# DanHelmy/hdr-realtime-video-pipeline

Hardware: AMD Instinct MI355X
Metric: frames/sec (HDRTVNet++ AGCM+LE+HG fp16 3840x2160 + fused RGB48 post into the pinned host ring); p50 per-frame ms in p50_ms (higher is better)
Workload: dtype f16

## Files before the change

### hdr-realtime-video-pipeline_amd/csrc/api_graph.hip

```cpp
#include "api.h"

namespace hdrtv_host {

void Seq::conv(const std::string &key, const f16 *src0, int c0, const f16 *src1, int c1, int Hi, int Wi, int act, int mode, f16 *dst, int dstC, int Hd, int Wd, const f16 *res1, const f16 *res2, f16 *dst_full, f16 *dst_planar, const f16 *res_planar, const float *dotw, float *dst_dot, int s0_stride)
{
    if (!ok()) return;
    auto it = c->conv.find(key);
    if (it == c->conv.end()) { rc = fail(c, HDRTV_ESTATE, "no packed conv %s", key.c_str()); return; }
    const ConvLayer &L = it->second;
    ConvParams p;
    memset(&p, 0, sizeof p);
    p.src0 = src0; p.src1 = src1; p.c0 = c0; p.c1 = c1;
    p.s0_stride = s0_stride ? s0_stride : c0; p.s1_stride = c1;
    p.Hi = Hi; p.Wi = Wi;
    const int pad = L.ks / 2;
    p.Ho = (Hi + 2 * pad - L.ks) / L.stride + 1;
    p.Wo = (Wi + 2 * pad - L.ks) / L.stride + 1;
    p.wpk = wtp<f16>(c, L.wpk); p.scale = wtp<float>(c, L.scale); p.shift = wtp<float>(c, L.shift);
    p.CoutPad = L.coutPad; p.Cout = L.cout; p.act = act; p.mode = mode;
    p.dst = dst; p.dst_full = dst_full; p.dstC = dstC; p.Hd = Hd; p.Wd = Wd;
    p.res1 = res1; p.res2 = res2; p.dst_planar = dst_planar; p.res_planar = res_planar;
    p.dotw = dotw; p.dst_dot = dst_dot;
    if (c0 + c1 != L.cin) { rc = fail(c, HDRTV_ESTATE, "conv %s: channel mismatch", key.c_str()); return; }
    p.zeros = wtp<f16>(c, c->zeros_off);
// ... 548 lines not shown
    }
    q.conv32("LE.up_conv3.0", t5, nullptr, "", s.H1, s.W1, ACT_RELU, ST_PS, up3, 32, H, W, fea0);
    q.conv32("LE.HR_conv2", up3, cond1, "LE.SFT_layer2", H, W, ACT_RELU, ST_NHWC, f0b, 32, H, W);
    q.conv32("LE.conv_last", f0b, nullptr, "", H, W, ACT_NONE, ST_PLANAR3, nullptr, 0, H, W, nullptr, nullptr, out_planar, img);
    return q.rc;
}

size_t hg_need_plan(hdrtv_ctx *c, int Hp, int Wp, HgNeedParams &p)
{
    memset(&p, 0, sizeof p);
    p.Hp = Hp; p.Wp = Wp;
    constexpr int n_layers = (int)(sizeof hg_layers / sizeof hg_layers[0]);
    static_assert(n_layers + 1 <= HG_NEED_MAX_LAYERS && n_layers + 3 <= HG_NEED_MAX_TENSORS, "hg_need's tables are too small");
    constexpr int max_level = [] { int m = 0; for (const HgLayer &L : hg_layers) m = L.level > m ? L.level : m; return m; }();
    static_assert(max_level < HG_NEED_LEVELS, "hg_need's unit tables have too few levels");
    memcpy(p.lu, hg_need_unit_log2[c->var.at("hg_sparse") == 1 ? 1 : 2], sizeof p.lu);
    auto ncell = [&](int level) { return (((Hp >> level) + 15) / 16) * (((Wp >> level) + 15) / 16); };
    auto nwords = [&](int level) {
        size_t m = 0;
        for (const auto &tab : hg_need_unit_log2) {
            const int u = 1 << tab[level], rows = std::max(((Hp >> level) + u - 1) / u, ((Hp >> level) + 7) / 8);
            m = std::max(m, (size_t)rows * ((((Wp >> level) + u - 1) / u + 63) / 64));
        }
        return m;
    };
    const char *names[HG_NEED_MAX_TENSORS];
    int level[HG_NEED_MAX_TENSORS], nt = 0;
    auto tensor = [&](const char *name, int lev) {
        if (!name) name = "part";
        for (int i = 0; i < nt; ++i)
            if (!strcmp(names[i], name)) return i;
        names[nt] = name; level[nt] = lev;
        return nt++;
    };
    for (int i = 0; i < n_layers; ++i) {
        const HgLayer &L = hg_layers[i];
        HgNeedLayer &N = p.L[i + 1];
        N.level = L.level; N.ks = L.ks; N.tw = 16;
        N.mode = L.mode == ST_POOL ? 1 : (L.ps ? 2 : 0);
        N.in = tensor(L.in, L.level);
        N.skip = L.skip ? tensor(L.skip, L.level) : -1;
        N.out = tensor(L.out, L.out_level());
        N.th = L.ks == 3 && Seq::prw_tile_rows(c, L.mode, L.cout, Hp >> L.level, Wp >> L.level) == 8 ? 8 : 16;
    }
    const int nt_table = nt;
    {
        HgNeedLayer &N = p.L[0];
        N.level = 0; N.ks = 3; N.mode = 1;
        N.out = tensor(hg_layers[0].in, 1);
        N.in = tensor("img", 0);
        N.skip = -1;
        N.th = 8; N.tw = 32;
    }
    p.n_layers = n_layers + 1;
    bool seen[HG_NEED_MAX_TENSORS] = {};
    for (int i = p.n_layers - 1; i >= 0; --i) {
        HgNeedLayer &N = p.L[i];
        N.in_first = !seen[N.in];
        seen[N.in] = true;
        if (N.skip >= 0) { N.skip_first = !seen[N.skip]; seen[N.skip] = true; }
    }
    size_t off = 0;
    auto take = [&](size_t bytes) { const size_t o = off; off = (off + bytes + 15) & ~(size_t)15; return (int)o; };
    p.flags_off = take((size_t)ncell(0));
    take((size_t)ncell(0));
    for (int t = 0; t < nt_table; ++t)
        if (strcmp(names[t], "part")) take((size_t)ncell(level[t]));
    for (int i = 1; i <= n_layers; ++i) p.L[i].list_off = take(4 * (2 * (size_t)ncell(p.L[i].level) + 4));
    size_t scratch = 0;
    for (int t = 0; t < nt; ++t) scratch = std::max(scratch, nwords(level[t]));
    for (int t = 0; t < nt_table; ++t) {
        p.map_off[t] = take(8 * nwords(level[t]));
        if (!strcmp(names[t], "part")) p.flags_map = t;
    }
    for (int i = 0; i < p.n_layers; ++i) {
        p.L[i].out_chained = i + 1 < p.n_layers ? p.L[i + 1].in == p.L[i].out : p.L[i].out == p.flags_map;
        p.L[i].in_chained = i > 0 && p.L[i - 1].out == p.L[i].in;
    }
    p.scratch_words = (int)scratch;
    p.kbits_off = take(8 * scratch);
    p.tbits_off = take(8 * scratch);
    p.L[0].list_off = take(4 * (2 * (size_t)ncell(0) + 4));
    p.map_off[nt_table] = take(8 * nwords(0));
    return off;
}

int run_hg(hdrtv_ctx *c, Seq &q, const f16 *base, void *out, int out_f32, bool complete_taps)
{
    const Shapes s = shapes_for(c->H, c->W);
    const int Hp = s.Hp, Wp = s.Wp;
    f16 *img = q.wsp<f16>("hg.img");
    uint8_t *mask = q.wsp<uint8_t>("hg.mask");
    const bool sparse = !complete_taps && c->var.at("hg_sparse") != 0 && !c->hg_i8 && !c->var.at("final_recompute");
    HgNeedParams np;
    if (sparse) {
        hg_need_plan(c, Hp, Wp, np);
        np.base = q.wsp<unsigned char>("hg.need");
    }
    if (q.ws == c->lane_ws[0] && !complete_taps) {
        hipStreamCaptureStatus cap = hipStreamCaptureStatusNone;
        c->taps_partial = sparse;
        c->taps_replayable = sparse && hipStreamIsCapturing(q.s, &cap) == hipSuccess && cap != hipStreamCaptureStatusNone;
        c->taps_stream = q.s;
    }
    if (!complete_taps)
        q.chk(hg_prep_launch(base, s.H, s.W, Hp, Wp, img, mask, c->mask_r, 0.1f, q.s, sparse ? np.base + np.flags_off : nullptr), "hg_prep",
              "hg_prep", 0.0, 13.0 * Hp * Wp);
    if (sparse) q.chk(hg_need_launch(np, q.s), "hg_need", "hg_need", 0.0, 0.0);
    float *part = q.wsp<float>("hg.part");
    const bool light = !c->var.at("final_recompute");
    float *part2 = light ? q.wsp<float>("hg.part2") : nullptr;
    const f16 *w2frag = light ? wtp<f16>(c, c->hgf_wfrag) + 6 * 64 * 8 : nullptr;
    constexpr int n_layers = (int)(sizeof hg_layers / sizeof hg_layers[0]);
    const char *tn[3 * n_layers];
    void *tp[3 * n_layers];
    int nt = 0;
    auto tensor = [&](const char *name) -> void * {
        if (!name) return nullptr;
        for (int i = 0; i < nt; ++i)
            if (!strcmp(tn[i], name)) return tp[i];
        char key[32];
        snprintf(key, sizeof key, "%s%s", c->hg_i8 ? "hg8." : "hg.", name);
        tn[nt] = name;
        tp[nt] = q.wsp<void>(key);
        return tp[nt++];
    };
    const bool c1_list = sparse && light;
    q.c3("hg.conv1", img, Hp, Wp, ACT_RELU, nullptr, (f16 *)tensor(hg_layers[0].in), c->hg_q0_inv, c->hg_q0_zero, w2frag, part2,
         c1_list ? reinterpret_cast<const int *>(np.base + np.L[0].list_off) : nullptr, c1_list ? ((Hp + 7) / 8) * ((Wp + 31) / 32) : 0);
    char key[32];
    for (const HgLayer &L : hg_layers) {
        snprintf(key, sizeof key, "hg.%s", L.name);
        if (sparse) {
            const HgNeedLayer &N = np.L[&L - hg_layers + 1];
            q.need_list = reinterpret_cast<const int *>(np.base + N.list_off);
            q.need_th = N.th;
            q.need_total = (((Hp >> L.level) + N.th - 1) / N.th) * (((Wp >> L.level) + 15) / 16);
        }
        const int c1 = L.skip_cin, c0 = L.cin - c1, Hi = Hp >> L.level, Wi = Wp >> L.level;
        const int Ho = Hp >> L.out_level(), Wo = Wp >> L.out_level();
        const bool dot3 = L.mode == ST_PS_DOT3;
        const float *dotw = dot3 ? wtp<float>(c, c->hg_w10a) : nullptr;
        float *dst_dot = dot3 ? part : nullptr;
        if (c->hg_i8)
            q.conv8(key, (const int8_t *)tensor(L.in), c0, (const int8_t *)tensor(L.skip), c1, Hi, Wi, L.mode, tensor(L.out), L.out_c(), Ho, Wo, dotw, dst_dot);
        else
            q.conv(key, (const f16 *)tensor(L.in), c0, (const f16 *)tensor(L.skip), c1, Hi, Wi, L.act, L.mode, (f16 *)tensor(L.out), L.out_c(), Ho, Wo,
                   nullptr, nullptr, nullptr, nullptr, nullptr, dotw, dst_dot);
    }
    if (!q.ok() || complete_taps) return q.rc;
    const C3Layer &L1 = c->c3.at("hg.conv1");
    HgFinalFusedArgs fa;
    fa.img = img; fa.mask = mask; fa.part = part; fa.wfrag = wtp<f16>(c, c->hgf_wfrag);
    fa.scale = wtp<float>(c, L1.scale); fa.shift = wtp<float>(c, L1.shift);
    fa.b10 = wtp<float>(c, c->f32v.at("hg.b10"));
    fa.wl = wtp<float>(c, c->f32v.at("hg.wl")); fa.bl = wtp<float>(c, c->f32v.at("hg.bl"));
    fa.out = out; fa.out_f32 = out_f32; fa.H = s.H; fa.W = s.W; fa.Hp = Hp; fa.Wp = Wp;
    if (light)
        q.chk(hg_final_light_launch(fa, part2, q.s), "hg_final", "hg_final_light", (double)s.H * s.W * 6 * 3,
              (double)s.H * s.W * (6 + 1 + 32 + 3 * (out_f32 ? 4 : 2)));
#ifdef HDRTV_AB
    else
        q.chk(hg_final_fused_launch(fa, c->n_cu, q.s), "hg_final", "hg_final_fused", (double)Hp * Wp * (128 * 3 + 6 * 3),
              (double)s.H * s.W * (6 + 1 + 16 + 3 * (out_f32 ? 4 : 2)));
#endif
    return q.rc;
}

}
```

### hdr-realtime-video-pipeline_amd/csrc/api_util.hip

```cpp
#include "api.h"

namespace hdrtv_host {

int fail(hdrtv_ctx *c, int code, const char *fmt, ...)
{
    char buf[512];
    va_list ap;
    va_start(ap, fmt);
    vsnprintf(buf, sizeof buf, fmt, ap);
    va_end(ap);
    if (c) { std::lock_guard<std::mutex> lk(c->err_mu); c->err = buf; }
    return code;
}

namespace {
const std::pair<const char *, int> k_variants[] = {
    {"le_rows", 1},
    {"le_rows_min", 8},
    {"le_rows_i8", 1},
    {"le_rows_fq", 1},
    {"prw", 1},
    {"prw_i8", 1},
    {"pglds_nt_slow", 3},
    {"no_t16", 0},
    {"conv32_old", 0},
    {"conv32_nosplit", 0},
    {"conv32_nw", 0},
    {"no_c3fuse", 0},
    {"no_c3q8", 0},
    {"glds1_old", 0},
    {"hg_sparse", 2},
    {"final_recompute", 0},
    {"cond3_fused", 1},
    {"cond2_fused", 1},
    {"pre_split", 0},
    {"force_ncu", 0},
    {"light_wgs", 2},
    {"f32_narrow_below", 0},
    {"f32_mfma", 1},
};
const char *const k_ab_only[] = {"conv32_old", "conv32_nosplit", "conv32_nw", "glds1_old", "final_recompute"};
}
bool variant_allowed(const std::string &name, int value)
{
#ifdef HDRTV_AB
    (void)name; (void)value;
    return true;
#else
    if (value == 0) return true;
    for (const char *n : k_ab_only) if (name == n) return false;
    return true;
#endif
}
void variants_init(hdrtv_ctx *c)
{
    for (const auto &kv : k_variants) c->var[kv.first] = kv.second;
    const char *e = getenv("HDRTV_VARIANTS");
    if (!e) return;
    std::string str(e);
    size_t pos = 0;
    while (pos < str.size()) {
        size_t nx = str.find(',', pos);
        if (nx == std::string::npos) nx = str.size();
        const std::string one = str.substr(pos, nx - pos);
        const size_t eq = one.find('=');
        if (eq != std::string::npos) {
            auto it = c->var.find(one.substr(0, eq));
            if (it != c->var.end() && variant_allowed(it->first, atoi(one.c_str() + eq + 1))) it->second = atoi(one.c_str() + eq + 1);
        }
        pos = nx + 1;
    }
}

}
```

### hdr-realtime-video-pipeline_amd/csrc/hg_need.hip

```cpp
#include "launchers.h"

namespace {

constexpr int NT = 1024, LDS_WORDS = 2304;
using u64 = unsigned long long;

__constant__ u64 k_tile_bits[5] = {~0ull, 0x5555555555555555ull, 0x1111111111111111ull, 0x0101010101010101ull, 0x0001000100010001ull};

struct Map {
    int h, w, nw;
};
__device__ __forceinline__ Map map_of(const HgNeedParams &p, int level)
{
    const int lu = p.lu[level], r = (1 << lu) - 1;
    Map m;
    m.h = ((p.Hp >> level) + r) >> lu;
    m.w = ((p.Wp >> level) + r) >> lu;
    m.nw = (m.w + 63) >> 6;
    return m;
}
__device__ __forceinline__ u64 word(const u64 *b, const Map &m, int y, int wi)
{
    return (unsigned)y < (unsigned)m.h && (unsigned)wi < (unsigned)m.nw ? b[y * m.nw + wi] : 0;
}
__device__ __forceinline__ u64 row_mask(int w, int wi)
{
    const int n = w - 64 * wi;
    return n >= 64 ? ~0ull : (n <= 0 ? 0ull : (1ull << n) - 1);
}
__device__ __forceinline__ u64 spread2(unsigned v)
{
    u64 x = v;
    x = (x | x << 16) & 0x0000FFFF0000FFFFull;
    x = (x | x << 8) & 0x00FF00FF00FF00FFull;
    x = (x | x << 4) & 0x0F0F0F0F0F0F0F0Full;
    x = (x | x << 2) & 0x3333333333333333ull;
    x = (x | x << 1) & 0x5555555555555555ull;
    return x | x << 1;
}
__device__ __forceinline__ unsigned pairs_any(u64 v)
{
    u64 x = (v | v >> 1) & 0x5555555555555555ull;
    x = (x | x >> 1) & 0x3333333333333333ull;
    x = (x | x >> 2) & 0x0F0F0F0F0F0F0F0Full;
    x = (x | x >> 4) & 0x00FF00FF00FF00FFull;
    x = (x | x >> 8) & 0x0000FFFF0000FFFFull;
    x = (x | x >> 16) & 0x00000000FFFFFFFFull;
    return (unsigned)x;
}

__global__ __launch_bounds__(NT) void hg_need_kernel(HgNeedParams p)
{
    __shared__ u64 s_k[LDS_WORDS], s_t[LDS_WORDS], s_n[LDS_WORDS];
    __shared__ int s_wave[NT / 64];
    const int tid = threadIdx.x;
    {
        const Map m = map_of(p, 0);
        const HgNeedLayer &L = p.L[p.n_layers - 1];
        u64 *fb = L.out_chained && m.h * m.nw <= LDS_WORDS ? s_n : reinterpret_cast<u64 *>(p.base + p.map_off[p.flags_map]);
        unsigned char *fl = p.base + p.flags_off;
        constexpr int NW = NT / 64, B = 8;
        const int lane = tid & 63, n0 = m.h * m.nw;
        for (int i0 = tid >> 6; i0 < n0; i0 += B * NW) {
            int at[B];
            unsigned char c[B];
#pragma unroll
            for (int j = 0; j < B; ++j) {
                const int i = i0 + j * NW, y = i / m.nw, x = 64 * (i - y * m.nw) + lane;
                at[j] = i < n0 && x < m.w ? y * m.w + x : -1;
                c[j] = at[j] >= 0 ? fl[at[j]] : 0;
            }
#pragma unroll
            for (int j = 0; j < B; ++j) {
                const u64 v = __ballot(c[j] != 0);
                if (at[j] >= 0) fl[at[j]] = 0;
                if (lane == 0 && i0 + j * NW < n0) fb[i0 + j * NW] = v;
            }
        }
    }
    __syncthreads();
    for (int li = p.n_layers - 1; li >= 0; --li) {
        const HgNeedLayer L = p.L[li];
        const int olev = L.level + (L.mode == 1 ? 1 : 0) - (L.mode == 2 ? 1 : 0);
        const Map mk = map_of(p, L.level), mo = map_of(p, olev);
        const int lu = p.lu[L.level], nk = mk.h * mk.nw;
        const int sh = p.lu[olev] - lu + olev - L.level;
        const int lth = L.th == 8 ? 3 : 4, ltw = L.tw == 32 ? 5 : 4, lbw = ltw - lu;
        const int ty_n = ((p.Hp >> L.level) + L.th - 1) >> lth, tx_n = ((p.Wp >> L.level) + (1 << ltw) - 1) >> ltw, nt = ty_n * mk.nw;
        const bool lds = max(nk, nt) <= LDS_WORDS;
        u64 *km = lds ? s_k : reinterpret_cast<u64 *>(p.base + p.kbits_off);
        u64 *tm = lds ? s_t : reinterpret_cast<u64 *>(p.base + p.tbits_off);
        const u64 *om = L.out_chained && mo.h * mo.nw <= LDS_WORDS ? s_n : reinterpret_cast<const u64 *>(p.base + p.map_off[L.out]);
        for (int i = tid; i < nk; i += NT) {
            const int y = i / mk.nw, wi = i - y * mk.nw;
            u64 k;
            if (sh == 0) {
                k = word(om, mo, y, wi);
            } else if (sh > 0) {
                k = spread2((unsigned)(word(om, mo, y >> 1, wi >> 1) >> (32 * (wi & 1))));
            } else {
                k = 0;
                for (int dy = 0; dy < 2; ++dy)
                    k |= (u64)pairs_any(word(om, mo, 2 * y + dy, 2 * wi)) | (u64)pairs_any(word(om, mo, 2 * y + dy, 2 * wi + 1)) << 32;
            }
            km[i] = k & row_mask(mk.w, wi);
        }
        __syncthreads();
        u64 *ig = reinterpret_cast<u64 *>(p.base + p.map_off[L.in]), *im = L.in_chained && nk <= LDS_WORDS ? s_n : ig;
        u64 *sm = L.skip >= 0 ? reinterpret_cast<u64 *>(p.base + p.map_off[L.skip]) : nullptr;
        for (int i = tid; i < nk; i += NT) {
            const int y = i / mk.nw, wi = i - y * mk.nw;
            u64 v = km[i];
            if (L.ks == 3) {
                for (int dy = -1; dy <= 1; ++dy) {
                    const u64 c = word(km, mk, y + dy, wi);
                    v |= c | c << 1 | c >> 1 | word(km, mk, y + dy, wi - 1) >> 63 | word(km, mk, y + dy, wi + 1) << 63;
                }
                v &= row_mask(mk.w, wi);
            }
            im[i] = L.in_first ? v : (ig[i] | v);
            if (sm) sm[i] = L.skip_first ? v : (sm[i] | v);
        }
        const int r_sh = lth - lu;
        for (int i = tid; i < nt; i += NT) {
            const int ty = i / mk.nw, wi = i - ty * mk.nw;
            const int r0 = r_sh >= 0 ? ty << r_sh : ty >> -r_sh, nr = r_sh >= 0 ? 1 << r_sh : 1;
            u64 v = 0;
            for (int r = r0; r < min(r0 + nr, mk.h); ++r) v |= km[r * mk.nw + wi];
            for (int s = 1; s < (1 << lbw); s <<= 1) v |= v >> s;
            tm[i] = v & k_tile_bits[lbw];
        }
        __syncthreads();
        const int per = (nt + NT - 1) / NT, c0 = tid * per, c1 = min(nt, c0 + per);
        int cnt = 0;
        for (int i = c0; i < c1; ++i) cnt += __popcll(tm[i]);
        int incl = cnt;
        for (int d = 1; d < 64; d <<= 1) {
            const int v = __shfl_up(incl, d, 64);
            if ((tid & 63) >= d) incl += v;
        }
        if ((tid & 63) == 63) s_wave[tid >> 6] = incl;
        __syncthreads();
        int o = incl - cnt, total = 0;
        for (int w = 0; w < NT / 64; ++w) {
            const int v = s_wave[w];
            if (w < (tid >> 6)) o += v;
            total += v;
        }
        int *lst = reinterpret_cast<int *>(p.base + L.list_off);
        if (tid == 0) lst[0] = total;
        for (int i = c0; i < c1; ++i) {
            const int ty = i / mk.nw, wi = i - ty * mk.nw;
            for (u64 v = tm[i]; v; v &= v - 1) lst[1 + o++] = ty * tx_n + ((64 * wi + __ffsll(v) - 1) >> lbw);
        }
    }
}

}

hipError_t hg_need_launch(const HgNeedParams &p, hipStream_t s)
{
    if (!p.base || p.n_layers < 1 || p.n_layers > HG_NEED_MAX_LAYERS) return hipErrorInvalidValue;
    for (int i = 0; i < p.n_layers; ++i) {
        const HgNeedLayer &L = p.L[i];
        const int olev = L.level + (L.mode == 1 ? 1 : 0) - (L.mode == 2 ? 1 : 0);
        if (L.level < 0 || L.level >= HG_NEED_LEVELS || olev < 0 || olev >= HG_NEED_LEVELS) return hipErrorInvalidValue;
        const int sh = p.lu[olev] - p.lu[L.level] + olev - L.level;
        if (p.lu[L.level] < 0 || p.lu[L.level] > 4 || sh < -1 || sh > 1 || (L.th != 8 && L.th != 16) ||
            (L.tw != 0 && L.tw != 16 && L.tw != 32))
            return hipErrorInvalidValue;
    }
    if (p.lu[0] != 4) return hipErrorInvalidValue;
    hipLaunchKernelGGL(hg_need_kernel, dim3(1), dim3(NT), 0, s, p);
    return hipGetLastError();
}
```

### hdr-realtime-video-pipeline_amd/csrc/launchers.h

```cpp
#pragma once
#include "common.h"

struct DevOnce {
    unsigned char set[64] = {};
    static int cur() { int d = 0; return hipGetDevice(&d) == hipSuccess && d >= 0 && d < 64 ? d : 0; }
    bool need() const { return !set[cur()]; }
    void done() { set[cur()] = 1; }
};
template <class K> hipError_t allow_lds(DevOnce &once, K kern, int bytes)
{
    if (!once.need()) return hipSuccess;
    const hipError_t e = hipFuncSetAttribute(reinterpret_cast<const void *>(kern), hipFuncAttributeMaxDynamicSharedMemorySize, bytes);
    if (e == hipSuccess) once.done();
    return e;
}

hipError_t conv_igemm_launch(ConvParams p, int cin_t, int bn, int ks, int stride, hipStream_t stream);
hipError_t conv_glds1_launch(ConvParams p, hipStream_t stream, int n_cu = 0, bool old_form = false, bool *list_taken = nullptr);
hipError_t conv_pglds_launch(ConvParams p, int n_cu, hipStream_t stream, bool *list_taken = nullptr);
hipError_t conv_prw_launch(ConvParams p, int th, int n_cu, hipStream_t stream, bool *list_taken = nullptr);
hipError_t conv_pglds_i8_launch(ConvI8Params p, int n_cu, hipStream_t stream);
hipError_t conv_prw_i8_launch(ConvI8Params p, int th, int n_cu, hipStream_t stream);
hipError_t conv1x1_i8_launch(ConvI8Params p, hipStream_t stream);
hipError_t conv32p_launch(Conv32Params p, int n_cu, hipStream_t stream, int nw = 0);
hipError_t conv32s_launch(Conv32Params p, int n_cu, hipStream_t stream, bool nosplit = false);
hipError_t le_rb_rows_launch(RowsRbParams p, int n_cu, hipStream_t stream);
hipError_t le_rb_rows_i8_launch(RowsRbI8Params p, int n_cu, hipStream_t stream);
hipError_t le_tail_rows_i8_launch(RowsTailI8Params p, int n_cu, hipStream_t stream);
hipError_t le_head_rows_i8_launch(RowsHeadI8Params p, int n_cu, hipStream_t stream);
hipError_t le_tail_rows_launch(RowsTailParams p, int n_cu, hipStream_t stream);
hipError_t le_head_rows_launch(RowsHeadParams p, int n_cu, hipStream_t stream);
hipError_t conv_t16_launch(ConvParams p, hipStream_t stream, int n_cu);
hipError_t conv_q8_launch(ConvQ8Params p, hipStream_t stream, int n_cu);
hipError_t conv_q8_multi_launch(ConvQ8MultiParams p, int n_cu, hipStream_t stream);
hipError_t conv3x3s2_preg_launch(ConvParams p, int n_cu, hipStream_t stream);

hipError_t pre_unpack_launch(const uint8_t *bgr, f16 *out, int H, int W, hipStream_t s);
hipError_t cond_resize_launch(const f16 *in, f16 *out, int H, int W, int Ho, int Wo, const float *wx, const int *xmn,
                              const int *xns, const float *wy, const int *ymn, const int *yns, hipStream_t s);
hipError_t pre_fused_launch(const uint8_t *bgr, f16 *out, f16 *cond, int H, int W, int Ho, int Wo, const float *wx, const int *xmn,
                            const int *xns, const float *wy, const int *ymn, const int *yns, int mode, hipStream_t s);
hipError_t post_u8_launch(const void *in, int is_f32, int H, int W, uint8_t *bgr, hipStream_t s);
hipError_t post_rgb48_launch(const void *in, int is_f32, int H, int W, uint16_t *rgb, int pq, float peak, hipStream_t s,
                             const float *pq_bnd = nullptr);

struct FakeQ { int on; float inv, zoff, scale, zero; };
hipError_t cls_block_launch(const void *in, int in_f16, int Ci, int Hi, int Wi, const float *nmean, const float *nrstd,
                            const float *ngamma, const float *nbeta, const float *Wt, const float *bias, int Co, float *out,
                            int Ho, int Wo, float *part, hipStream_t s, const FakeQ *qin = nullptr, const FakeQ *qstat = nullptr,
                            int *nblk = nullptr);
hipError_t cls_stats_launch(const float *part, int C, int nblk, int n, float eps, float *mean, float *rstd, hipStream_t s);
struct AgcmFoldArgs {
    const float *mean5;
    const float *w20, *b20;
    const float *ws[3], *bs[3], *wt[3], *bt[3];
    const float *w1, *b1, *w2, *b2, *w3, *b3;
};
hipError_t agcm_fold_launch(const AgcmFoldArgs &a, f16 *frags, float *biasbuf, hipStream_t s);
hipError_t agcm_mlp_launch(const f16 *in, f16 *out, size_t npix, const f16 *frags, const float *biasbuf, hipStream_t s);

hipError_t conv_c3_launch(const f16 *in, int H, int W, const f16 *wfrag, const float *scale, const float *shift, int cout,
                          int act, f16 *out, f16 *out_pool, int n_cu, hipStream_t s, float pool_q_inv = 0.f, float pool_q_zero = 0.f,
                          const f16 *w2frag = nullptr, float *part2 = nullptr,
                          const int *tile_list = nullptr, bool *list_taken = nullptr);
hipError_t conv_c3_q8_launch(const f16 *in, int H, int W, const int8_t *wq, const float *scale, const float *shift, float q_inv,
                             float q_zoff, int act, f16 *out, int n_cu, hipStream_t s);
struct QLastArgs {
    const int8_t *wq;
    const float *ss;
    float q_inv, q_zoff;
};
hipError_t le_cond_trunk_launch(const f16 *img, int H, int W, const f16 *wfrag, const float *bias, f16 *cond, f16 *cond1,
                                int n_cu, hipStream_t s, const QLastArgs *q6 = nullptr);
hipError_t cond_tail_launch(const f16 *x, int x_stride, size_t npx, const f16 *wfrag, const float *bias, f16 *out, int n_cu,
                            hipStream_t s, const QLastArgs *q2 = nullptr);
struct TrunkQ8Args {
    const int8_t *wfrag;
    const float *consts;
    float q1_inv, q1_zoff, q4_inv;
    float zoff[5];
};
hipError_t le_cond_trunk_q8_launch(const f16 *img, int H, int W, const TrunkQ8Args &a, f16 *cond, f16 *cond1, int n_cu, hipStream_t s);
hipError_t cond_tail_q8_launch(const int8_t *x, size_t npx, const int8_t *wfrag, const float *consts, float zoff2, f16 *out, int n_cu,
                               hipStream_t s);
hipError_t agcm_mlp_q8_launch(const f16 *in, f16 *out, size_t npix, const int8_t *wfrag, const float *consts, float q1_inv, float q1_zoff,
                              float zoff2, float zoff3, hipStream_t s);
hipError_t planar3_to_q8_launch(const f16 *in, size_t npix, float inv, float zoff, int8_t *out, hipStream_t s);
struct AgcmFoldQ8Args {
    FakeQ q20, qlin[6];
    const float *P, *Q;
    float inv2, inv3;
    float *consts;
};
hipError_t agcm_fold_q8_launch(const AgcmFoldArgs &a, const AgcmFoldQ8Args &q, float *biasbuf, hipStream_t s);
hipError_t hg_prep_launch(const f16 *base, int H, int W, int Hp, int Wp, f16 *img_pad, uint8_t *mask, float r, float thresh,
                          hipStream_t s, uint8_t *flags = nullptr);
constexpr int HG_NEED_MAX_LAYERS = 24, HG_NEED_MAX_TENSORS = 32, HG_NEED_LEVELS = 6;
constexpr int hg_need_unit_log2[3][HG_NEED_LEVELS] = {{4, 4, 4, 4, 4, 4}, {4, 4, 4, 4, 4, 4}, {4, 2, 1, 0, 0, 0}};
struct HgNeedLayer {
    int level, mode, ks;
    int in, skip, out;
    int in_first, skip_first;
    int out_chained;
    int in_chained;
    int th, tw;
    int list_off;
};
struct HgNeedParams {
    unsigned char *base;
    int Hp, Wp, n_layers;
    int lu[HG_NEED_LEVELS];
    int flags_off;
    int flags_map;
    int kbits_off, tbits_off, scratch_words;
    int map_off[HG_NEED_MAX_TENSORS];
    HgNeedLayer L[HG_NEED_MAX_LAYERS];
};
hipError_t hg_need_launch(const HgNeedParams &p, hipStream_t s);
struct HgFinalFusedArgs {
    const f16 *img;
    const uint8_t *mask;
    const float *part;
    const f16 *wfrag;
    const float *scale, *shift, *b10, *wl, *bl;
    void *out;
    int out_f32, H, W, Hp, Wp;
};
hipError_t hg_final_fused_launch(const HgFinalFusedArgs &a, int n_cu, hipStream_t s);
hipError_t hg_final_light_launch(const HgFinalFusedArgs &a, const float *part2, hipStream_t s);
hipError_t letterbox_launch(const LetterboxParams &p, hipStream_t s);
hipError_t post_scale_launch(const PostScaleParams &p, int is_f32, int pq, hipStream_t s);
hipError_t post_scale_ar_launch(const PostScaleParams &p, int antiring, int is_f32, int pq, hipStream_t s);
hipError_t post_scale_cas_launch(const PostScaleParams &p, int antiring, int cas, int is_f32, int pq, hipStream_t s);
hipError_t post_fsr_launch(const PostFsrParams &p, int rcas, float sharp, int is_f32, int pq, hipStream_t s);
hipError_t post_ycbcr10_launch(const Ycbcr10Params &p, int is_f32, int pq, hipStream_t s);
hipError_t rgb48_to_ycbcr10_launch(const Ycbcr10Params &p, hipStream_t s);
hipError_t post_ycbcr10_dither_launch(const Ycbcr10Params &p, int is_f32, int pq, hipStream_t s);
hipError_t rgb48_to_ycbcr10_dither_launch(const Ycbcr10Params &p, hipStream_t s);
hipError_t rgb48_deband_launch(const DebandParams &p, hipStream_t s);
hipError_t light_stats_launch(const LightStatsParams &p, int is_f32, int pq, int max_wgs, hipStream_t s);
hipError_t rgb48_light_stats_launch(const LightStatsParams &p, int max_wgs, hipStream_t s);
hipError_t metrics_launch(const MetricsParams &p, hipStream_t s);
int metrics_blocks(int H, int W);

hipError_t conv_f32_launch(const F32ConvParams &p, int ks, int stride, int n_cu, hipStream_t s);
bool conv_f32_on_mfma(const F32ConvParams &p, int ks, int n_cu);
hipError_t ew_f32_launch(int op, const float *a, const float *b, const float *c, float *y, size_t n, hipStream_t s);
hipError_t avgpool3s2_leaky_f32_launch(const float *x, float *y, int C, int H, int W, float slope, hipStream_t s);
hipError_t instnorm_f32_launch(float *x, const float *gamma, const float *beta, int C, int n, float eps, hipStream_t s);
hipError_t plane_mean_f32_launch(const float *x, float *y, int C, int n, hipStream_t s);
hipError_t gfm_heads_f32_launch(const F32GfmParams &p, hipStream_t s);
hipError_t maxpool2_f32_launch(const float *x, float *y, int C, int H, int W, hipStream_t s);
hipError_t window_f32_launch(const float *x, float *y, int C, int H, int W, int Ho, int Wo, int mode, hipStream_t s);
hipError_t hg_mask_f32_launch(const float *base, float *mask, size_t npix, float r, hipStream_t s);
hipError_t hg_blend_f32_launch(const float *t, const float *img, const float *mask, float *out, int H, int W, int Hp, int Wp,
                               hipStream_t s);
hipError_t pre_f32_launch(const uint8_t *bgr, float *rgb, float *cond, int H, int W, int Ho, int Wo, const float *wx,
                          const int *xmn, const int *xns, const float *wy, const int *ymn, const int *yns, int mode, hipStream_t s);
```

Baseline: 150.1.

## Add all-LDS variant of the HG sparsity need planner kernel

```diff
diff --git a/hdr-realtime-video-pipeline_amd/csrc/api_graph.hip b/hdr-realtime-video-pipeline_amd/csrc/api_graph.hip
--- a/hdr-realtime-video-pipeline_amd/csrc/api_graph.hip
+++ b/hdr-realtime-video-pipeline_amd/csrc/api_graph.hip
@@ -654,6 +654,8 @@
     p.tbits_off = take(8 * scratch);
     p.L[0].list_off = take(4 * (2 * (size_t)ncell(0) + 4));
     p.map_off[nt_table] = take(8 * nwords(0));
+    p.lds = hg_need_lds_layout(p);
+    if (!c->var.at("hg_need_lds")) p.lds.fits = 0;
     return off;
 }
 
@@ -668,6 +670,7 @@
     if (sparse) {
         hg_need_plan(c, Hp, Wp, np);
         np.base = q.wsp<unsigned char>("hg.need");
+        if ((reinterpret_cast<uintptr_t>(np.base) | (unsigned)np.flags_off) & 15) np.lds.fits = 0;
     }
     if (q.ws == c->lane_ws[0] && !complete_taps) {
         hipStreamCaptureStatus cap = hipStreamCaptureStatusNone;
@@ -678,7 +681,7 @@
     if (!complete_taps)
         q.chk(hg_prep_launch(base, s.H, s.W, Hp, Wp, img, mask, c->mask_r, 0.1f, q.s, sparse ? np.base + np.flags_off : nullptr), "hg_prep",
               "hg_prep", 0.0, 13.0 * Hp * Wp);
-    if (sparse) q.chk(hg_need_launch(np, q.s), "hg_need", "hg_need", 0.0, 0.0);
+    if (sparse) q.chk(hg_need_launch(np, q.s), "hg_need", np.lds.fits ? "hg_need<lds>" : "hg_need", 0.0, 0.0);
     float *part = q.wsp<float>("hg.part");
     const bool light = !c->var.at("final_recompute");
     float *part2 = light ? q.wsp<float>("hg.part2") : nullptr;
diff --git a/hdr-realtime-video-pipeline_amd/csrc/api_util.hip b/hdr-realtime-video-pipeline_amd/csrc/api_util.hip
--- a/hdr-realtime-video-pipeline_amd/csrc/api_util.hip
+++ b/hdr-realtime-video-pipeline_amd/csrc/api_util.hip
@@ -30,6 +30,7 @@
     {"no_c3q8", 0},
     {"glds1_old", 0},
     {"hg_sparse", 2},
+    {"hg_need_lds", 1},
     {"final_recompute", 0},
     {"cond3_fused", 1},
     {"cond2_fused", 1},
diff --git a/hdr-realtime-video-pipeline_amd/csrc/hg_need.hip b/hdr-realtime-video-pipeline_amd/csrc/hg_need.hip
--- a/hdr-realtime-video-pipeline_amd/csrc/hg_need.hip
+++ b/hdr-realtime-video-pipeline_amd/csrc/hg_need.hip
@@ -1,27 +1,23 @@
+#include <cstring>
+
 #include "launchers.h"
 
 namespace {
 
 constexpr int NT = 1024, LDS_WORDS = 2304;
 using u64 = unsigned long long;
+using Map = HgNeedMap;
+typedef __attribute__((address_space(3))) u64 *lds64_t;
+typedef __attribute__((address_space(3))) int *lds32_t;
 
 __constant__ u64 k_tile_bits[5] = {~0ull, 0x5555555555555555ull, 0x1111111111111111ull, 0x0101010101010101ull, 0x0001000100010001ull};
 
-struct Map {
-    int h, w, nw;
-};
-__device__ __forceinline__ Map map_of(const HgNeedParams &p, int level)
-{
-    const int lu = p.lu[level], r = (1 << lu) - 1;
-    Map m;
-    m.h = ((p.Hp >> level) + r) >> lu;
-    m.w = ((p.Wp >> level) + r) >> lu;
-    m.nw = (m.w + 63) >> 6;
-    return m;
-}
-__device__ __forceinline__ u64 word(const u64 *b, const Map &m, int y, int wi)
-{
-    return (unsigned)y < (unsigned)m.h && (unsigned)wi < (unsigned)m.nw ? b[y * m.nw + wi] : 0;
+__device__ __forceinline__ Map map_of(const HgNeedParams &p, int level) { return hg_need_map(p.Hp, p.Wp, p.lu[level], level); }
+template <class P> __device__ __forceinline__ u64 word(P b, const Map &m, int y, int wi)
+{
+    const bool in = (unsigned)y < (unsigned)m.h && (unsigned)wi < (unsigned)m.nw;
+    const u64 v = b[in ? y * m.nw + wi : 0];
+    return in ? v : 0;
 }
 __device__ __forceinline__ u64 row_mask(int w, int wi)
 {
@@ -49,6 +45,83 @@
     return (unsigned)x;
 }
 
+template <class P> __device__ __forceinline__ u64 k_word(P om, const Map &mo, const Map &mk, int sh, int y, int wi)
+{
+    u64 k;
+    if (sh == 0) {
+        k = word(om, mo, y, wi);
+    } else if (sh > 0) {
+        k = spread2((unsigned)(word(om, mo, y >> 1, wi >> 1) >> (32 * (wi & 1))));
+    } else {
+        k = (u64)pairs_any(word(om, mo, 2 * y, 2 * wi) | word(om, mo, 2 * y + 1, 2 * wi)) |
+            (u64)pairs_any(word(om, mo, 2 * y, 2 * wi + 1) | word(om, mo, 2 * y + 1, 2 * wi + 1)) << 32;
+    }
+    return k & row_mask(mk.w, wi);
+}
+template <class P> __device__ __forceinline__ u64 read_word(P km, const Map &mk, int ks, int y, int wi)
+{
+    u64 v = km[y * mk.nw + wi];
+    if (ks == 3) {
+        u64 c = 0, l = 0, r = 0;
+        const bool has_l = wi > 0, has_r = wi + 1 < mk.nw;
+#pragma unroll
+        for (int dy = -1; dy <= 1; ++dy) {
+            const bool in = (unsigned)(y + dy) < (unsigned)mk.h;
+            const int at = (in ? y + dy : y) * mk.nw + wi;
+            const u64 cc = km[at], ll = km[has_l ? at - 1 : at], rr = km[has_r ? at + 1 : at];
+            c |= in ? cc : 0;
+            l |= in && has_l ? ll : 0;
+            r |= in && has_r ? rr : 0;
+        }
+        v |= c | c << 1 | c >> 1 | l >> 63 | r << 63;
+        v &= row_mask(mk.w, wi);
+    }
+    return v;
+}
+template <class P> __device__ __forceinline__ u64 tile_word(P km, const Map &mk, int r_sh, int lbw, u64 low, int ty, int wi)
+{
+    const int r0 = r_sh >= 0 ? ty << r_sh : ty >> -r_sh, nr = r_sh >= 0 ? 1 << r_sh : 1;
+    u64 v = 0;
+    const int r1 = min(r0 + nr, mk.h);
+    for (int r = r0; r < r1; r += 4) {
+        u64 w[4];
+#pragma unroll
+        for (int j = 0; j < 4; ++j) w[j] = km[min(r + j, mk.h - 1) * mk.nw + wi];
+#pragma unroll
+        for (int j = 0; j < 4; ++j) v |= r + j < r1 ? w[j] : 0;
+    }
+    for (int s = 1; s < (1 << lbw); s <<= 1) v |= v >> s;
+    return v & low;
+}
+__device__ __forceinline__ int div_mul(int d) { return d > 1 ? (int)(0xFFFFFFFFu / (unsigned)d + 1) : 0; }
+__device__ __forceinline__ int div_by(int i, int d_mul) { return d_mul ? (int)__umulhi((unsigned)i, (unsigned)d_mul) : i; }
+template <int B, bool CLEAR, class P> __device__ __forceinline__ bool flags_to_map(const HgNeedParams &p, const Map &m, P fb, int tid)
+{
+    unsigned char *fl = p.base + p.flags_off;
+    constexpr int NW = NT / 64;
+    const int lane = tid & 63, n0 = m.h * m.nw, dv = div_mul(m.nw);
+    bool any = false;
+    for (int i0 = __builtin_amdgcn_readfirstlane(tid >> 6); i0 < n0; i0 += B * NW) {
+        int at[B];
+        unsigned char c[B];
+#pragma unroll
+        for (int j = 0; j < B; ++j) {
+            const int i = i0 + j * NW, y = div_by(i, dv), x = 64 * (i - y * m.nw) + lane;
+            at[j] = i < n0 && x < m.w ? y * m.w + x : -1;
+            const unsigned char b = fl[max(at[j], 0)];
+            c[j] = at[j] >= 0 ? b : 0;
+        }
+#pragma unroll
+        for (int j = 0; j < B; ++j) {
+            const u64 v = __ballot(c[j] != 0);
+            if (CLEAR && at[j] >= 0) fl[at[j]] = 0;
+            if (lane == 0 && i0 + j * NW < n0) fb[i0 + j * NW] = v;
+            any = any || v != 0;
+        }
+    }
+    return any;
+}
+
 __global__ __launch_bounds__(NT) void hg_need_kernel(HgNeedParams p)
 {
     __shared__ u64 s_k[LDS_WORDS], s_t[LDS_WORDS], s_n[LDS_WORDS];
@@ -58,77 +131,38 @@
         const Map m = map_of(p, 0);
         const HgNeedLayer &L = p.L[p.n_layers - 1];
         u64 *fb = L.out_chained && m.h * m.nw <= LDS_WORDS ? s_n : reinterpret_cast<u64 *>(p.base + p.map_off[p.flags_map]);
-        unsigned char *fl = p.base + p.flags_off;
-        constexpr int NW = NT / 64, B = 8;
-        const int lane = tid & 63, n0 = m.h * m.nw;
-        for (int i0 = tid >> 6; i0 < n0; i0 += B * NW) {
-            int at[B];
-            unsigned char c[B];
-#pragma unroll
-            for (int j = 0; j < B; ++j) {
-                const int i = i0 + j * NW, y = i / m.nw, x = 64 * (i - y * m.nw) + lane;
-                at[j] = i < n0 && x < m.w ? y * m.w + x : -1;
-                c[j] = at[j] >= 0 ? fl[at[j]] : 0;
-            }
-#pragma unroll
-            for (int j = 0; j < B; ++j) {
-                const u64 v = __ballot(c[j] != 0);
-                if (at[j] >= 0) fl[at[j]] = 0;
-                if (lane == 0 && i0 + j * NW < n0) fb[i0 + j * NW] = v;
-            }
-        }
+        flags_to_map<8, true>(p, m, fb, tid);
     }
     __syncthreads();
     for (int li = p.n_layers - 1; li >= 0; --li) {
         const HgNeedLayer L = p.L[li];
-        const int olev = L.level + (L.mode == 1 ? 1 : 0) - (L.mode == 2 ? 1 : 0);
+        const int olev = hg_need_olev(L.level, L.mode);
         const Map mk = map_of(p, L.level), mo = map_of(p, olev);
         const int lu = p.lu[L.level], nk = mk.h * mk.nw;
         const int sh = p.lu[olev] - lu + olev - L.level;
-        const int lth = L.th == 8 ? 3 : 4, ltw = L.tw == 32 ? 5 : 4, lbw = ltw - lu;
-        const int ty_n = ((p.Hp >> L.level) + L.th - 1) >> lth, tx_n = ((p.Wp >> L.level) + (1 << ltw) - 1) >> ltw, nt = ty_n * mk.nw;
+        const HgNeedTiles T = hg_need_tiles(p.Hp, p.Wp, L.level, L.th, L.tw);
+        const int lbw = T.ltw - lu, tx_n = T.tx_n, nt = T.ty_n * mk.nw;
         const bool lds = max(nk, nt) <= LDS_WORDS;
         u64 *km = lds ? s_k : reinterpret_cast<u64 *>(p.base + p.kbits_off);
         u64 *tm = lds ? s_t : reinterpret_cast<u64 *>(p.base + p.tbits_off);
         const u64 *om = L.out_chained && mo.h * mo.nw <= LDS_WORDS ? s_n : reinterpret_cast<const u64 *>(p.base + p.map_off[L.out]);
         for (int i = tid; i < nk; i += NT) {
             const int y = i / mk.nw, wi = i - y * mk.nw;
-            u64 k;
-            if (sh == 0) {
-                k = word(om, mo, y, wi);
-            } else if (sh > 0) {
-                k = spread2((unsigned)(word(om, mo, y >> 1, wi >> 1) >> (32 * (wi & 1))));
-            } else {
-                k = 0;
-                for (int dy = 0; dy < 2; ++dy)
-                    k |= (u64)pairs_any(word(om, mo, 2 * y + dy, 2 * wi)) | (u64)pairs_any(word(om, mo, 2 * y + dy, 2 * wi + 1)) << 32;
-            }
-            km[i] = k & row_mask(mk.w, wi);
+            km[i] = k_word(om, mo, mk, sh, y, wi);
         }
         __syncthreads();
         u64 *ig = reinterpret_cast<u64 *>(p.base + p.map_off[L.in]), *im = L.in_chained && nk <= LDS_WORDS ? s_n : ig;
         u64 *sm = L.skip >= 0 ? reinterpret_cast<u64 *>(p.base + p.map_off[L.skip]) : nullptr;
         for (int i = tid; i < nk; i += NT) {
             const int y = i / mk.nw, wi = i - y * mk.nw;
-            u64 v = km[i];
-            if (L.ks == 3) {
-                for (int dy = -1; dy <= 1; ++dy) {
-                    const u64 c = word(km, mk, y + dy, wi);
-                    v |= c | c << 1 | c >> 1 | word(km, mk, y + dy, wi - 1) >> 63 | word(km, mk, y + dy, wi + 1) << 63;
-                }
-                v &= row_mask(mk.w, wi);
-            }
+            const u64 v = read_word(km, mk, L.ks, y, wi);
             im[i] = L.in_first ? v : (ig[i] | v);
             if (sm) sm[i] = L.skip_first ? v : (sm[i] | v);
         }
-        const int r_sh = lth - lu;
+        const int r_sh = T.lth - lu;
         for (int i = tid; i < nt; i += NT) {
             const int ty = i / mk.nw, wi = i - ty * mk.nw;
-            const int r0 = r_sh >= 0 ? ty << r_sh : ty >> -r_sh, nr = r_sh >= 0 ? 1 << r_sh : 1;
-            u64 v = 0;
-            for (int r = r0; r < min(r0 + nr, mk.h); ++r) v |= km[r * mk.nw + wi];
-            for (int s = 1; s < (1 << lbw); s <<= 1) v |= v >> s;
-            tm[i] = v & k_tile_bits[lbw];
+            tm[i] = tile_word(km, mk, r_sh, lbw, k_tile_bits[lbw], ty, wi);
         }
         __syncthreads();
         const int per = (nt + NT - 1) / NT, c0 = tid * per, c1 = min(nt, c0 + per);
@@ -156,6 +190,160 @@
     }
 }
 
+enum { R_MK_H, R_MK_W, R_MK_NW, R_MO_H, R_MO_W, R_MO_NW, R_SH, R_KS, R_LBW, R_RSH, R_TXN, R_NT, R_IN_SRC, R_IN_STORE, R_SKIP_DST,
+       R_TB, R_LIST, R_DIV, R_NK, R_N };
+static_assert(R_N <= HG_NEED_LDS_REC_INTS, "a layer record outgrew its LDS block");
+__device__ __forceinline__ int uni(int v) { return __builtin_amdgcn_readfirstlane(v); }
+__device__ __forceinline__ u64 tile_fields_low(int lbw)
+{
+    u64 m = 1;
+    for (int f = 1 << lbw; f < 64; f <<= 1) m |= m << f;
+    return m;
+}
+__device__ __forceinline__ u64 tiles_packed(u64 v, int lbw)
+{
+    for (int s = 0; s < lbw; ++s) v = pairs_any(v);
+    return v;
+}
+
+__global__ __launch_bounds__(NT) void hg_need_lds_kernel(HgNeedParams p)
+{
+    extern __shared__ __attribute__((aligned(16))) u64 smem[];
+    const lds64_t lds = (lds64_t)smem;
+    const lds64_t s_k = lds + p.lds.k_off, s_n = lds + p.lds.n_off;
+    const lds32_t s_pre = (lds32_t)(lds + p.lds.pre_off), s_rec = (lds32_t)(lds + p.lds.rec_off), s_wave = (lds32_t)(lds + p.lds.wave_off);
+    const int tid = threadIdx.x, lane = tid & 63, wave = uni(tid >> 6), n_layers = p.n_layers;
+    HgNeedLayer L = {};
+    int in_slot = -1, skip_slot = -1, tb_off = 0;
+    if (tid < n_layers) {
+        L = p.L[tid];
+        in_slot = p.lds.in_slot[tid]; skip_slot = p.lds.skip_slot[tid]; tb_off = p.lds.tb_off[tid];
+    }
+    const Map m0 = map_of(p, 0);
+    const bool any = flags_to_map<36, false>(p, m0, s_n, tid);
+    if (tid < n_layers) {
+        const int olev = hg_need_olev(L.level, L.mode);
+        int lu = p.lu[0], luo = p.lu[0];
+#pragma unroll
+        for (int k = 1; k < HG_NEED_LEVELS; ++k) {
+            lu = L.level == k ? p.lu[k] : lu;
+            luo = olev == k ? p.lu[k] : luo;
+        }
+        const Map mk = hg_need_map(p.Hp, p.Wp, lu, L.level), mo = hg_need_map(p.Hp, p.Wp, luo, olev);
+        const HgNeedTiles T = hg_need_tiles(p.Hp, p.Wp, L.level, L.th, L.tw);
+        int in_src = -1, skip_dst = -1;
+#pragma unroll
+        for (int k = 0; k < HG_NEED_LDS_SKIPS; ++k) {
+            in_src = in_slot == k ? p.lds.skip_off[k] : in_src;
+            skip_dst = skip_slot == k ? p.lds.skip_off[k] : skip_dst;
+        }
+        const lds32_t r = s_rec + tid * HG_NEED_LDS_REC_INTS;
+        r[R_MK_H] = mk.h; r[R_MK_W] = mk.w; r[R_MK_NW] = mk.nw;
+        r[R_MO_H] = mo.h; r[R_MO_W] = mo.w; r[R_MO_NW] = mo.nw;
+        r[R_SH] = luo - lu + olev - L.level;
+        r[R_KS] = L.ks;
+        r[R_LBW] = T.ltw - lu;
+        r[R_RSH] = T.lth - lu;
+        r[R_TXN] = T.tx_n;
+        r[R_NT] = T.ty_n * mk.nw;
+        r[R_IN_SRC] = in_src;
+        r[R_IN_STORE] = L.in_chained;
+        r[R_SKIP_DST] = skip_dst;
+        r[R_TB] = tb_off;
+        r[R_LIST] = L.list_off;
+        r[R_DIV] = div_mul(mk.nw);
+        r[R_NK] = mk.h * mk.nw;
+    }
+    if (lane == 0) s_wave[wave] = any;
+    __syncthreads();
+    int flagged = 0;
+#pragma unroll
+    for (int w = 0; w < NT / 64; ++w) flagged |= s_wave[w];
+    if (!uni(flagged)) {
+        if (tid < n_layers) *reinterpret_cast<int *>(p.base + s_rec[tid * HG_NEED_LDS_REC_INTS + R_LIST]) = 0;
+        return;
+    }
+    for (int li = n_layers - 1; li >= 0; --li) {
+        const lds32_t r = s_rec + li * HG_NEED_LDS_REC_INTS;
+        Map mk, mo;
+        mk.h = uni(r[R_MK_H]); mk.w = uni(r[R_MK_W]); mk.nw = uni(r[R_MK_NW]);
+        mo.h = uni(r[R_MO_H]); mo.w = uni(r[R_MO_W]); mo.nw = uni(r[R_MO_NW]);
+        const int sh = uni(r[R_SH]), ks = uni(r[R_KS]), lbw = uni(r[R_LBW]), r_sh = uni(r[R_RSH]), nt = uni(r[R_NT]), nk = uni(r[R_NK]);
+        const int in_src = uni(r[R_IN_SRC]), in_store = uni(r[R_IN_STORE]), skip_dst = uni(r[R_SKIP_DST]), dv = uni(r[R_DIV]);
+        const lds64_t tb = lds + uni(r[R_TB]);
+        const u64 low = tile_fields_low(lbw);
+        for (int i = tid; i < nk; i += NT) {
+            const int y = div_by(i, dv), wi = i - y * mk.nw;
+            s_k[i] = k_word(s_n, mo, mk, sh, y, wi);
+        }
+        __syncthreads();
+        for (int i = tid; i < nk; i += NT) {
+            const int y = div_by(i, dv), wi = i - y * mk.nw;
+            const u64 v = read_word(s_k, mk, ks, y, wi);
+            if (in_store) s_n[i] = in_src >= 0 ? (lds[in_src + i] | v) : v;
+            if (skip_dst >= 0) lds[skip_dst + i] = v;
+        }
+        for (int i = tid; i < nt; i += NT) {
+            const int ty = div_by(i, dv), wi = i - ty * mk.nw;
+            tb[i] = tiles_packed(tile_word(s_k, mk, r_sh, lbw, low, ty, wi), lbw);
+        }
+        __syncthreads();
+    }
+    {
+        uint4 *fl = reinterpret_cast<uint4 *>(p.base + p.flags_off);
+        const int n16 = (m0.h * m0.w + 15) >> 4;
+        for (int i = tid; i < n16; i += NT) fl[i] = make_uint4(0, 0, 0, 0);
+    }
+    const int tb0 = p.lds.tb_off[0], n_tb = p.lds.tb_off[n_layers] - tb0;
+    const lds64_t tball = lds + tb0;
+    {
+        const int per = (n_tb + NT - 1) / NT, c0 = tid * per, c1 = min(n_tb, c0 + per);
+        int cnt = 0;
+        for (int i = c0; i < c1; ++i) cnt += __popcll(tball[i]);
+        int incl = cnt;
+        for (int d = 1; d < 64; d <<= 1) {
+            const int v = __shfl_up(incl, d, 64);
+            if (lane >= d) incl += v;
+        }
+        if (lane == 63) s_wave[wave] = incl;
+        __syncthreads();
+        int o = incl - cnt, total = 0;
+#pragma unroll
+        for (int w = 0; w < NT / 64; ++w) {
+            const int v = s_wave[w];
+            if (w < wave) o += v;
+            total += v;
+        }
+        for (int i = c0; i < c1; ++i) {
+            s_pre[i] = o;
+            o += __popcll(tball[i]);
+        }
+        if (tid == 0) s_pre[n_tb] = total;
+    }
+    __syncthreads();
+    if (tid < n_layers) {
+        const lds32_t r = s_rec + tid * HG_NEED_LDS_REC_INTS;
+        const int w0 = r[R_TB] - tb0;
+        *reinterpret_cast<int *>(p.base + r[R_LIST]) = s_pre[w0 + r[R_NT]] - s_pre[w0];
+    }
+    int turn = 0;
+    for (int li = 0; li < n_layers; ++li) {
+        const lds32_t r = s_rec + li * HG_NEED_LDS_REC_INTS;
+        const int nw = uni(r[R_MK_NW]), lbw = uni(r[R_LBW]), tx_n = uni(r[R_TXN]), nt = uni(r[R_NT]), dv = uni(r[R_DIV]);
+        const int w0 = uni(r[R_TB]) - tb0, q = 6 - lbw, steps = (nt + (1 << lbw) - 1) >> lbw;
+        int *lst = reinterpret_cast<int *>(p.base + uni(r[R_LIST])) + 1;
+        const int base = s_pre[w0], sub = lane >> q, bit = lane & ((1 << q) - 1);
+        for (int st = (wave - turn) & (NT / 64 - 1); st < steps; st += NT / 64) {
+            const int i = (st << lbw) + sub;
+            const u64 v = i < nt ? tball[w0 + i] : 0;
+            if (!(v >> bit & 1)) continue;
+            const int ty = div_by(i, dv), wi = i - ty * nw;
+            lst[s_pre[w0 + i] - base + __popcll(v & ((1ull << bit) - 1))] = ty * tx_n + (wi << q) + bit;
+        }
+        turn = (turn + steps) & (NT / 64 - 1);
+    }
+}
+
 }
 
 hipError_t hg_need_launch(const HgNeedParams &p, hipStream_t s)
@@ -163,7 +351,7 @@
     if (!p.base || p.n_layers < 1 || p.n_layers > HG_NEED_MAX_LAYERS) return hipErrorInvalidValue;
     for (int i = 0; i < p.n_layers; ++i) {
         const HgNeedLayer &L = p.L[i];
-        const int olev = L.level + (L.mode == 1 ? 1 : 0) - (L.mode == 2 ? 1 : 0);
+        const int olev = hg_need_olev(L.level, L.mode);
         if (L.level < 0 || L.level >= HG_NEED_LEVELS || olev < 0 || olev >= HG_NEED_LEVELS) return hipErrorInvalidValue;
         const int sh = p.lu[olev] - p.lu[L.level] + olev - L.level;
         if (p.lu[L.level] < 0 || p.lu[L.level] > 4 || sh < -1 || sh > 1 || (L.th != 8 && L.th != 16) ||
@@ -171,6 +359,18 @@
             return hipErrorInvalidValue;
     }
     if (p.lu[0] != 4) return hipErrorInvalidValue;
-    hipLaunchKernelGGL(hg_need_kernel, dim3(1), dim3(NT), 0, s, p);
+    bool lds = p.lds.fits != 0 && ((reinterpret_cast<uintptr_t>(p.base) | (unsigned)p.flags_off) & 15) == 0;
+    if (lds) {
+        const HgNeedLds d = hg_need_lds_layout(p);
+        lds = d.fits && memcmp(&d, &p.lds, sizeof d) == 0;
+    }
+    if (lds) {
+        static DevOnce once;
+        const hipError_t e = allow_lds(once, hg_need_lds_kernel, HG_NEED_LDS_BYTES);
+        if (e != hipSuccess) return e;
+        hipLaunchKernelGGL(hg_need_lds_kernel, dim3(1), dim3(NT), (size_t)p.lds.words * 8, s, p);
+    } else {
+        hipLaunchKernelGGL(hg_need_kernel, dim3(1), dim3(NT), 0, s, p);
+    }
     return hipGetLastError();
 }
diff --git a/hdr-realtime-video-pipeline_amd/csrc/hg_need_plan.h b/hdr-realtime-video-pipeline_amd/csrc/hg_need_plan.h
--- /dev/null
+++ b/hdr-realtime-video-pipeline_amd/csrc/hg_need_plan.h
@@ -0,0 +1,134 @@
+#pragma once
+
+#if defined(__HIPCC__)
+#define HG_NEED_FN __host__ __device__ __forceinline__
+#else
+#define HG_NEED_FN inline
+#endif
+
+constexpr int HG_NEED_MAX_LAYERS = 24, HG_NEED_MAX_TENSORS = 32, HG_NEED_LEVELS = 6;
+constexpr int hg_need_unit_log2[3][HG_NEED_LEVELS] = {{4, 4, 4, 4, 4, 4}, {4, 4, 4, 4, 4, 4}, {4, 2, 1, 0, 0, 0}};
+struct HgNeedLayer {
+    int level, mode, ks;
+    int in, skip, out;
+    int in_first, skip_first;
+    int out_chained;
+    int in_chained;
+    int th, tw;
+    int list_off;
+};
+
+constexpr int HG_NEED_LDS_BYTES = 160 * 1024, HG_NEED_LDS_SKIPS = 4, HG_NEED_LDS_REC_INTS = 20, HG_NEED_LDS_WAVES = 16;
+struct HgNeedLds {
+    int fits;
+    int k_off, n_off;
+    int n_skip, skip_tensor[HG_NEED_LDS_SKIPS], skip_off[HG_NEED_LDS_SKIPS + 1];
+    int in_slot[HG_NEED_MAX_LAYERS], skip_slot[HG_NEED_MAX_LAYERS];
+    int tb_off[HG_NEED_MAX_LAYERS + 1];
+    int pre_off, rec_off, wave_off, words;
+};
+struct HgNeedParams {
+    unsigned char *base;
+    int Hp, Wp, n_layers;
+    int lu[HG_NEED_LEVELS];
+    int flags_off;
+    int flags_map;
+    int kbits_off, tbits_off, scratch_words;
+    int map_off[HG_NEED_MAX_TENSORS];
+    HgNeedLayer L[HG_NEED_MAX_LAYERS];
+    HgNeedLds lds;
+};
+
+struct HgNeedMap {
+    int h, w, nw;
+};
+HG_NEED_FN HgNeedMap hg_need_map(int Hp, int Wp, int l, int level)
+{
+    const int r = (1 << l) - 1;
+    HgNeedMap m;
+    m.h = ((Hp >> level) + r) >> l;
+    m.w = ((Wp >> level) + r) >> l;
+    m.nw = (m.w + 63) >> 6;
+    return m;
+}
+HG_NEED_FN int hg_need_olev(int level, int mode) { return level + (mode == 1 ? 1 : 0) - (mode == 2 ? 1 : 0); }
+struct HgNeedTiles {
+    int lth, ltw, ty_n, tx_n;
+};
+HG_NEED_FN HgNeedTiles hg_need_tiles(int Hp, int Wp, int level, int th, int tw)
+{
+    HgNeedTiles t;
+    t.lth = th == 8 ? 3 : 4;
+    t.ltw = tw == 32 ? 5 : 4;
+    t.ty_n = ((Hp >> level) + th - 1) >> t.lth;
+    t.tx_n = ((Wp >> level) + (1 << t.ltw) - 1) >> t.ltw;
+    return t;
+}
+
+HG_NEED_FN HgNeedLds hg_need_lds_layout(const HgNeedParams &p)
+{
+    HgNeedLds d;
+    d.fits = 0;
+    d.k_off = d.n_off = d.n_skip = d.pre_off = d.rec_off = d.wave_off = d.words = 0;
+    for (int s = 0; s < HG_NEED_LDS_SKIPS; ++s) d.skip_tensor[s] = -1, d.skip_off[s] = 0;
+    d.skip_off[HG_NEED_LDS_SKIPS] = 0;
+    for (int i = 0; i < HG_NEED_MAX_LAYERS; ++i) d.in_slot[i] = d.skip_slot[i] = -1, d.tb_off[i] = 0;
+    d.tb_off[HG_NEED_MAX_LAYERS] = 0;
+    if (p.n_layers < 1 || p.n_layers > HG_NEED_MAX_LAYERS) return d;
+    const long long limit = HG_NEED_LDS_BYTES / 8;
+    auto words = [&](int level) { const HgNeedMap m = hg_need_map(p.Hp, p.Wp, p.lu[level], level); return (long long)m.h * m.nw; };
+    bool chain = true;
+    long long work = words(0), off = 0;
+    long long skip_words[HG_NEED_LDS_SKIPS] = {};
+    for (int i = p.n_layers - 1; i >= 0; --i) {
+        const HgNeedLayer &L = p.L[i];
+        const int olev = hg_need_olev(L.level, L.mode);
+        if (L.level < 0 || L.level >= HG_NEED_LEVELS || olev < 0 || olev >= HG_NEED_LEVELS) return d;
+        chain = chain && L.out_chained && (i == 0 ? L.in_first != 0 : L.in_chained != 0);
+        const long long k = words(L.level), o = words(olev);
+        work = k > work ? k : work;
+        work = o > work ? o : work;
+        if (L.skip >= 0) {
+            chain = chain && L.skip_first && d.n_skip < HG_NEED_LDS_SKIPS;
+            if (!chain) return d;
+            d.skip_tensor[d.n_skip] = L.skip;
+            skip_words[d.n_skip] = k;
+            d.skip_slot[i] = d.n_skip++;
+        }
+        if (!L.in_first) {
+            for (int s = 0; s < d.n_skip; ++s)
+                if (d.skip_tensor[s] == L.in && skip_words[s] == k) d.in_slot[i] = s;
+            chain = chain && d.in_slot[i] >= 0;
+        }
+        if (!chain || work > limit) return d;
+    }
+    d.k_off = 0;
+    d.n_off = (int)work;
+    off = 2 * work;
+    for (int s = 0; s < d.n_skip; ++s) {
+        d.skip_off[s] = (int)off;
+        off += skip_words[s];
+        if (off > limit) return d;
+    }
+    for (int s = d.n_skip; s <= HG_NEED_LDS_SKIPS; ++s) d.skip_off[s] = (int)off;
+    for (int i = 0; i < p.n_layers; ++i) {
+        const HgNeedLayer &L = p.L[i];
+        d.tb_off[i] = (int)off;
+        off += (long long)hg_need_tiles(p.Hp, p.Wp, L.level, L.th, L.tw).ty_n * hg_need_map(p.Hp, p.Wp, p.lu[L.level], L.level).nw;
+        if (off > limit) return d;
+    }
+    for (int i = p.n_layers; i <= HG_NEED_MAX_LAYERS; ++i) d.tb_off[i] = (int)off;
+    const long long tbw = off - d.tb_off[0];
+    d.pre_off = (int)off;
+    off += (tbw + 1 + 1) / 2;
+    d.rec_off = (int)off;
+    off += ((long long)p.n_layers * HG_NEED_LDS_REC_INTS + 1) / 2;
+    d.wave_off = (int)off;
+    off += HG_NEED_LDS_WAVES / 2;
+    if (off > limit) return d;
+    d.words = (int)off;
+    d.fits = 1;
+    return d;
+}
+
+#undef HG_NEED_FN
diff --git a/hdr-realtime-video-pipeline_amd/csrc/launchers.h b/hdr-realtime-video-pipeline_amd/csrc/launchers.h
--- a/hdr-realtime-video-pipeline_amd/csrc/launchers.h
+++ b/hdr-realtime-video-pipeline_amd/csrc/launchers.h
@@ -1,5 +1,6 @@
 #pragma once
 #include "common.h"
+#include "hg_need_plan.h"
 
 struct DevOnce {
     unsigned char set[64] = {};
@@ -95,27 +96,6 @@
 hipError_t agcm_fold_q8_launch(const AgcmFoldArgs &a, const AgcmFoldQ8Args &q, float *biasbuf, hipStream_t s);
 hipError_t hg_prep_launch(const f16 *base, int H, int W, int Hp, int Wp, f16 *img_pad, uint8_t *mask, float r, float thresh,
                           hipStream_t s, uint8_t *flags = nullptr);
-constexpr int HG_NEED_MAX_LAYERS = 24, HG_NEED_MAX_TENSORS = 32, HG_NEED_LEVELS = 6;
-constexpr int hg_need_unit_log2[3][HG_NEED_LEVELS] = {{4, 4, 4, 4, 4, 4}, {4, 4, 4, 4, 4, 4}, {4, 2, 1, 0, 0, 0}};
-struct HgNeedLayer {
-    int level, mode, ks;
-    int in, skip, out;
-    int in_first, skip_first;
-    int out_chained;
-    int in_chained;
-    int th, tw;
-    int list_off;
-};
-struct HgNeedParams {
-    unsigned char *base;
-    int Hp, Wp, n_layers;
-    int lu[HG_NEED_LEVELS];
-    int flags_off;
-    int flags_map;
-    int kbits_off, tbits_off, scratch_words;
-    int map_off[HG_NEED_MAX_TENSORS];
-    HgNeedLayer L[HG_NEED_MAX_LAYERS];
-};
 hipError_t hg_need_launch(const HgNeedParams &p, hipStream_t s);
 struct HgFinalFusedArgs {
     const f16 *img;
```

Result: no change. 151.5 (median of 6 runs) (+0.9%).
